# quantumjot/sequitr

Hardware: AMD Instinct MI355X
Metric: segmented Mpixels/sec on 512x512 tiles; IoU vs reference (higher is better)
Workload: dtype f32; 1 GPU; U-Net 2-class inference, launches of 32 512x512x1 tiles, fp32 (BASELINE.json configs[1]: filters 16-32-64-128-256, eltwise_mul bridge); logits + uint8 argmax mask; one 32-tile batch per GPU per step; tiles_this_rank=32

## Files before the change

include/sequitr_hip.h:

```cpp
#ifndef SEQUITR_HIP_H
#define SEQUITR_HIP_H

#include <stdint.h>

#ifdef __cplusplus
extern "C" {
#endif

#define SQ_OK 0
#define SQ_EINVAL (-1)
#define SQ_ELAUNCH (-2)
#define SQ_EALIGN (-3)

#define SQ_ACT_NONE 0
#define SQ_ACT_RELU 1
#define SQ_ACT_LEAKY 2

#define SQ_BRIDGE_NONE 0
#define SQ_BRIDGE_ADD 1
#define SQ_BRIDGE_MUL 2
#define SQ_BRIDGE_SUB 3

int sq_version(void);
const char *sq_last_error(void);
// ... 276 lines not shown

int64_t sq_weightmap_workspace(int N, int H, int W);
int sq_edt_sq_f32(const float *img, int32_t *d2, void *workspace, int N, int H, int W, void *stream);
int sq_weightmap_edt_f32(const float *img, double *out64, float *out32, void *workspace, int N, int H, int W,
                         double w0, double sigma, void *stream);

int64_t sq_weightmap2_workspace(int N, int H, int W);
int sq_wm2_boundary_points_u8(const float *img, uint8_t *points, int N, int H, int W, void *stream);
int64_t sq_delaunay2d_batch_i32(const int32_t *xy, const int64_t *offsets, int nsets, int32_t *simplices, double *longest,
                                int64_t cap);
int sq_weightmap2_delaunay_f32(const float *img, const int32_t *simplices, const double *longest, int nsimp, double *out64,
                               float *out32, void *workspace, int N, int H, int W, double w0, double sigma, void *stream);

int sq_pixelnorm_fwd_bf16(const void *x, void *y, int64_t npix, int C, float eps, void *stream);
int sq_pixelnorm_bwd_bf16(const void *x, const void *dy, void *dx, int64_t npix, int C, float eps, int act, void *stream);
int sq_pixelnorm_bwd2_bf16(const void *x, const void *g, const void *v, void *dg, void *dx2, int64_t npix, int C, float eps,
                           void *stream);
int sq_sumpool2x2_bf16(const void *x, void *y, int N, int H, int W, int C, float scale, void *stream);
int sq_broadcast2x2_bf16(const void *src, void *dst, int N, int H, int W, int C, float scale, void *stream);
int sq_broadcast2x2_act_bwd_bf16(const void *src, const void *gate, void *dst, int N, int H, int W, int C, float scale,
                                 int act, void *stream);
int sq_act_fwd_bf16(const void *x, void *y, int64_t n, int act, void *stream);
int sq_conv1x1_smallin_fwd_bf16(const float *x, const float *w, const float *bias, void *y, int64_t npix, int Ca, int C,
                                float wscale, int act, void *stream);
int sq_conv1x1_smallout_fwd_bf16(const void *x, const float *w, const float *bias, float *y, int64_t npix, int C, int Co,
                                 float wscale, int act, void *stream);
int64_t sq_wgrad1x1_small_workspace_bf16(int64_t npix, int Ca, int C);
int sq_wgrad1x1_small_bf16(const float *a, const void *b, float *m, float *asum, float *workspace, int64_t npix, int Ca,
                           int C, float scale, void *stream);
int sq_conv2d_nhwc_fwd_avgpool_bf16(const void *x, const void *wp, const float *bias, void *y, void *ypool, int N, int H, int W,
                                    int Cin, int Cout, int act, void *stream);
int sq_conv2d_nhwc_fwd_pixelnorm_bf16(const void *x, const void *wp, const float *bias, void *y, void *ynorm, int N, int H, int W,
                                      int Cin, int Cout, int act, float eps, void *stream);
int sq_conv2d_nhwc_dgrad_actgate_bf16(const void *dy, const void *wp_t, const void *gate, int act, void *dx, int N, int H,
                                      int W, int Cin, int Cout, int K, void *stream);
int sq_conv2d_nhwc_mosaic_bf16(const void *x, const void *wp, const float *bias, const void *gate, void *y, int Nimg, int h,
                               int w, int Cin, int Cout, int act, int R, int Cc, float *workspace, int64_t workspace_bytes,
                               void *stream);
#define SQ_PLAN_BF16 0
#define SQ_PLAN_MIXED 1
#define SQ_PLAN_F32 2
#define SQ_PLAN_PLAIN 0
#define SQ_PLAN_JUNCTION 1
#define SQ_PLAN_POOL 2
#define SQ_PLAN_MASK 3
#define SQ_PLAN_MASKGATE 4
#define SQ_PLAN_ACTGATE 5
#define SQ_PLAN_FIRSTBLOCK 8
#define SQ_PLAN_PIXELNORM 9
#define SQ_PLAN_CONCAT 10
#define SQ_PLAN_WSCALE 1
int sq_conv_plan(int family, int form, int N, int H, int W, int Cin, int Cout, int K, int act, int flags, const int *mosaic,
                 int64_t workspace_bytes, int *out);
int sq_conv2d_nhwc_wgrad_scaled_bf16(const void *x, const void *dy, float *dw, float *db, float *workspace, int N, int H,
                                     int W, int Cin, int Cout, int K, float dw_scale, void *stream);
int sq_conv2d_nhwc_wgrad_mosaic_bf16(const void *x, const void *dy, float *dw, float *db, float *workspace, int Nimg, int h,
                                     int w, int Cin, int Cout, int R, int Cc, float dw_scale, void *stream);

typedef struct sq_wgrad_item {
    const void *x, *dy;
    float *dw, *db;
    int32_t N, H, W, Cin, Cout, K;
    int32_t convT_cout;
    float dw_scale;
    int32_t accumulate;
    int32_t mosaic_R, mosaic_Cc;
    int32_t reserved;
} sq_wgrad_item;
int64_t sq_conv2d_nhwc_wgrad_group_workspace_bf16(const sq_wgrad_item *items, int n);
int sq_conv2d_nhwc_wgrad_group_bf16(const sq_wgrad_item *items, int n, float *workspace, void *stream);

#define SQ_WGP_KS 0
#define SQ_WGP_NI 1
#define SQ_WGP_NO 2
#define SQ_WGP_KIND 3
#define SQ_WGP_PF 4
#define SQ_WGP_NPAIRS 5
#define SQ_WGP_GX 6
#define SQ_WGP_TPB 7
#define SQ_WGP_G 8
#define SQ_WGP_WS 9
#define SQ_WGP_N 10
#define SQ_WGP_GROUP_N (SQ_WGP_N + 3)
#define SQ_WGP_PLAIN 0
#define SQ_WGP_MOSAIC 1
#define SQ_WGP_RAGGED 2
#define SQ_WGP_CONVT 3
#define SQ_WGP_F32 4
#define SQ_WGP_F32_SMALL 5
int sq_wgrad_plan(int family, int N, int H, int W, int Cin, int Cout, int K, const int *mosaic, int convT_cout, int64_t *out);
int sq_wgrad_group_plan(const sq_wgrad_item *items, int n, int64_t *out);

#define SQ_C3P_KIND 0
#define SQ_C3P_BN 1
#define SQ_C3P_KC 2
#define SQ_C3P_GX 3
#define SQ_C3P_GY 4
#define SQ_C3P_ADDR 5
#define SQ_C3P_N 6
#define SQ_C3_MFMA 0
#define SQ_C3_DIRECT 1
#define SQ_C3_FLAT 0
#define SQ_C3_WINDOW 1
int sq_conv3d_plan(int N, int D, int H, int W, int Cin, int Cout, int *out);
int sq_conv3d_ndhwc_fwd_f32(const float *x, const float *w, const float *bias, float *y, int N, int D, int H, int W,
                            int Cin, int Cout, int act, void *stream);
// ... 20 lines not shown
```

sequitr_amd/_lib.py:

```python
import ctypes
import os

_HERE = os.path.dirname(os.path.abspath(__file__))
LIB_PATH = os.path.join(_HERE, "_build", "libsequitr_hip.so")

c_void_p, c_int, c_float, c_int64 = ctypes.c_void_p, ctypes.c_int, ctypes.c_float, ctypes.c_int64


class WgradItem(ctypes.Structure):
    _fields_ = [("x", c_void_p), ("dy", c_void_p), ("dw", c_void_p), ("db", c_void_p),
                ("N", ctypes.c_int32), ("H", ctypes.c_int32), ("W", ctypes.c_int32), ("Cin", ctypes.c_int32),
                ("Cout", ctypes.c_int32), ("K", ctypes.c_int32), ("convT_cout", ctypes.c_int32), ("dw_scale", c_float),
                ("accumulate", ctypes.c_int32), ("mosaic_R", ctypes.c_int32), ("mosaic_Cc", ctypes.c_int32),
                ("reserved", ctypes.c_int32)]

SIGNATURES = {
    "sq_version": (c_int, []),
    "sq_last_error": (ctypes.c_char_p, []),
    "sq_conv2d_nhwc_fwd_f32": (c_int, [c_void_p] * 4 + [c_int] * 6 + [c_float, c_int, c_void_p]),
    "sq_maxpool2x2_fwd_f32": (c_int, [c_void_p] * 2 + [c_int] * 4 + [c_void_p]),
    "sq_avgpool2x2_fwd_f32": (c_int, [c_void_p] * 2 + [c_int] * 4 + [c_void_p]),
    "sq_convT2x2s2_nhwc_fwd_f32": (c_int, [c_void_p] * 5 + [c_int] * 6 + [c_void_p]),
    "sq_bridge_fwd_f32": (c_int, [c_void_p] * 3 + [c_int64, c_int, c_void_p]),
    "sq_conv1x1_argmax_fwd_f32": (c_int, [c_void_p] * 5 + [c_int] * 5 + [c_void_p]),
# ... 93 lines not shown
    "sq_conv2d_nhwc_wgrad_workspace_mixed_f32": (c_int64, [c_int] * 6),
    "sq_conv2d_nhwc_wgrad_mixed_f32": (c_int, [c_void_p] * 5 + [c_int] * 6 + [c_void_p]),
    "sq_conv2d_nhwc_wgrad_scaled_mixed_f32": (c_int, [c_void_p] * 5 + [c_int] * 6 + [c_float, c_void_p]),
    "sq_conv2d_nhwc_wgrad_scaled_f32": (c_int, [c_void_p] * 5 + [c_int] * 6 + [c_float, c_void_p]),
    "sq_conv3x3_first_fwd_bf16": (c_int, [c_void_p] * 4 + [c_int] * 6 + [c_void_p]),
    "sq_conv2d_nhwc_wgrad_workspace_bf16": (c_int64, [c_int] * 6),
    "sq_conv2d_nhwc_wgrad_bf16": (c_int, [c_void_p] * 5 + [c_int] * 6 + [c_void_p]),
    "sq_convT2x2s2_wgrad_bf16": (c_int, [c_void_p] * 5 + [c_int] * 5 + [c_void_p]),
    "sq_cast_f32_to_bf16": (c_int, [c_void_p] * 2 + [c_int64, c_void_p]),
    "sq_cast_bf16_to_f32": (c_int, [c_void_p] * 2 + [c_int64, c_void_p]),
    "sq_head_concat_fwd_bf16": (c_int, [c_void_p] * 3 + [c_int64, c_int, c_void_p]),
    "sq_head_concat_bwd_bf16": (c_int, [c_void_p] * 3 + [c_int64, c_int, c_void_p]),
    "sq_maxpool2x2_fwd_bf16": (c_int, [c_void_p] * 2 + [c_int] * 4 + [c_void_p]),
    "sq_maxpool2x2_bwd_bf16": (c_int, [c_void_p] * 3 + [c_int] * 4 + [c_void_p]),
    "sq_conv_pack_weights_multi_bf16": (c_int, [c_void_p, c_void_p, c_void_p, c_int, c_int, c_void_p]),
    "sq_conv_pack_weights_multi_scaled_bf16": (c_int, [c_void_p] * 4 + [c_int, c_int, c_void_p]),
    "sq_conv2d_nhwc_fwd_dropout_bf16": (c_int, [c_void_p] * 4 + [c_int] * 7 + [c_float, ctypes.c_uint32, c_void_p, c_void_p]),
    "sq_conv3x3_first_fwd_mask_bf16": (c_int, [c_void_p] * 5 + [c_int] * 6 + [c_void_p]),
    "sq_conv2d_nhwc_fwd_mask_bf16": (c_int, [c_void_p] * 5 + [c_int] * 7 + [c_void_p]),
    "sq_conv2d_nhwc_dgrad_maskgate_bf16": (c_int, [c_void_p] * 3 + [c_float, c_void_p] + [c_int] * 6 + [c_void_p]),
    "sq_conv2d_nhwc_wgrad_mixed_mosaic_f32": (c_int, [c_void_p] * 5 + [c_int] * 7 + [c_float, c_void_p]),
    "sq_conv2d_nhwc_mixed_mosaic_f32": (c_int, [c_void_p] * 5 + [c_int] * 8 + [c_void_p]),
    "sq_conv2d_nhwc_dgrad_actgate_mixed_f32": (c_int, [c_void_p] * 3 + [c_int, c_void_p] + [c_int] * 6 + [c_void_p]),
    "sq_conv2d_nhwc_fwd_dropout_pool_bf16": (c_int, [c_void_p] * 5 + [c_int] * 7 + [c_float, ctypes.c_uint32, c_void_p, c_void_p]),
    "sq_conv3x3_first_block_dropout_pool_bf16": (c_int, [c_void_p] * 9 + [c_int] * 3 + [c_float, ctypes.c_uint32, c_void_p, c_void_p]),
    "sq_relu_scale_bwd_bf16": (c_int, [c_void_p] * 3 + [c_int64, c_float, c_void_p]),
    "sq_bridge_bwd_s2d_bf16": (c_int, [c_void_p] * 5 + [c_int] * 5 + [c_void_p]),
    "sq_maxpool2x2_bwd_add_bf16": (c_int, [c_void_p] * 4 + [c_int] * 4 + [c_void_p]),
    "sq_maxpool2x2_bwd_add_gate_bf16": (c_int, [c_void_p] * 4 + [c_int] * 4 + [c_float, c_void_p]),
    "sq_conv2d_nhwc_dgrad_gate_bf16": (c_int, [c_void_p] * 3 + [c_float, c_void_p] + [c_int] * 6 + [c_void_p]),
    "sq_conv2d_nhwc_dgrad_junction_bf16": (c_int, [c_void_p] * 6 + [c_int] * 7 + [c_void_p]),
    "sq_conv1x1_head_bwd_gate_bf16": (c_int, [c_void_p] * 7 + [c_int64, c_int, c_int, c_float, c_void_p]),
    "sq_conv1x1_head_wce_fwd_bf16": (c_int, [c_void_p] * 7 + [c_int64, c_int, c_int, c_void_p]),
    "sq_conv1x1_head_wce_bwd_bf16": (c_int, [c_void_p] * 10 + [c_int64, c_int, c_int, c_float, c_void_p]),
    "sq_conv1x1_head_wce_bwd_loss_bf16": (c_int, [c_void_p] * 12 + [c_int64, c_int, c_int, c_float, c_void_p]),
    "sq_act_dropout_bwd_bf16": (c_int, [c_void_p] * 4 + [c_int64, c_float, c_int, c_void_p]),
    "sq_conv2d_nhwc_dgrad_relu_bf16": (c_int, [c_void_p] * 4 + [c_int] * 6 + [c_void_p]),
    "sq_pixelnorm_fwd_bf16": (c_int, [c_void_p] * 2 + [c_int64, c_int, c_float, c_void_p]),
    "sq_pixelnorm_bwd_bf16": (c_int, [c_void_p] * 3 + [c_int64, c_int, c_float, c_int, c_void_p]),
    "sq_pixelnorm_bwd2_bf16": (c_int, [c_void_p] * 5 + [c_int64, c_int, c_float, c_void_p]),
    "sq_sumpool2x2_bf16": (c_int, [c_void_p] * 2 + [c_int] * 4 + [c_float, c_void_p]),
    "sq_broadcast2x2_bf16": (c_int, [c_void_p] * 2 + [c_int] * 4 + [c_float, c_void_p]),
    "sq_broadcast2x2_act_bwd_bf16": (c_int, [c_void_p] * 3 + [c_int] * 4 + [c_float, c_int, c_void_p]),
    "sq_act_fwd_bf16": (c_int, [c_void_p] * 2 + [c_int64, c_int, c_void_p]),
    "sq_conv1x1_smallin_fwd_bf16": (c_int, [c_void_p] * 4 + [c_int64, c_int, c_int, c_float, c_int, c_void_p]),
    "sq_conv1x1_smallout_fwd_bf16": (c_int, [c_void_p] * 4 + [c_int64, c_int, c_int, c_float, c_int, c_void_p]),
    "sq_wgrad1x1_small_workspace_bf16": (c_int64, [c_int64, c_int, c_int]),
    "sq_wgrad1x1_small_bf16": (c_int, [c_void_p] * 5 + [c_int64, c_int, c_int, c_float, c_void_p]),
    "sq_conv2d_nhwc_fwd_avgpool_bf16": (c_int, [c_void_p] * 5 + [c_int] * 6 + [c_void_p]),
    "sq_conv2d_nhwc_fwd_pixelnorm_bf16": (c_int, [c_void_p] * 5 + [c_int] * 6 + [c_float, c_void_p]),
    "sq_conv2d_nhwc_dgrad_actgate_bf16": (c_int, [c_void_p] * 3 + [c_int, c_void_p] + [c_int] * 6 + [c_void_p]),
    "sq_conv2d_nhwc_mosaic_bf16": (c_int, [c_void_p] * 5 + [c_int] * 8 + [c_void_p, c_int64, c_void_p]),
    "sq_conv_plan": (c_int, [c_int] * 10 + [c_void_p, c_int64, c_void_p]),
    "sq_conv2d_nhwc_wgrad_scaled_bf16": (c_int, [c_void_p] * 5 + [c_int] * 6 + [c_float, c_void_p]),
    "sq_conv2d_nhwc_wgrad_mosaic_bf16": (c_int, [c_void_p] * 5 + [c_int] * 7 + [c_float, c_void_p]),
    "sq_conv2d_nhwc_wgrad_group_workspace_bf16": (c_int64, [c_void_p, c_int]),
    "sq_conv2d_nhwc_wgrad_group_bf16": (c_int, [c_void_p, c_int, c_void_p, c_void_p]),
    "sq_wgrad_plan": (c_int, [c_int] * 7 + [c_void_p, c_int, c_void_p]),
    "sq_wgrad_group_plan": (c_int, [c_void_p, c_int, c_void_p]),
    "sq_conv3d_plan": (c_int, [c_int] * 6 + [c_void_p]),
    "sq_conv3d_ndhwc_fwd_f32": (c_int, [c_void_p] * 4 + [c_int] * 7 + [c_void_p]),
    "sq_maxpool2x2x2_fwd_f32": (c_int, [c_void_p] * 2 + [c_int] * 5 + [c_void_p]),
    "sq_convT2x2x2s2_ndhwc_fwd_f32": (c_int, [c_void_p] * 5 + [c_int] * 7 + [c_void_p]),
    "sq_act_bwd_bf16": (c_int, [c_void_p] * 3 + [c_int64, c_int, c_void_p]),
    "sq_bridge_fwd_bf16": (c_int, [c_void_p] * 3 + [c_int64, c_int, c_void_p]),
    "sq_bridge_bwd_bf16": (c_int, [c_void_p] * 5 + [c_int64, c_int, c_void_p]),
    "sq_dropout_fwd_bf16": (c_int, [c_void_p] * 3 + [c_int64, c_float, ctypes.c_uint32, c_int, c_void_p, c_void_p]),
    "sq_dropout_bwd_bf16": (c_int, [c_void_p] * 3 + [c_int64, c_float, c_void_p]),
    "sq_convT2x2s2_nhwc_fwd_bf16": (c_int, [c_void_p] * 5 + [c_int] * 6 + [c_void_p]),
    "sq_convT2x2s2_bridge_both_fwd_bf16": (c_int, [c_void_p] * 6 + [c_int] * 6 + [c_void_p]),
    "sq_conv1x1_head_fwd_bf16": (c_int, [c_void_p] * 5 + [c_int64, c_int, c_int, c_void_p]),
    "sq_conv1x1_head_bwd_workspace_bf16": (c_int64, [c_int64, c_int, c_int]),
    "sq_conv1x1_head_bwd_bf16": (c_int, [c_void_p] * 7 + [c_int64, c_int, c_int, c_void_p]),
    "sq_conv3x3_first_wgrad_workspace_bf16": (c_int64, [c_int] * 5),
    "sq_conv3x3_first_wgrad_bf16": (c_int, [c_void_p] * 5 + [c_int] * 5 + [c_void_p]),
}

_lib = None


class SequitrHipError(RuntimeError):
    pass


def load():
    global _lib
    if _lib is not None:
        return _lib
    if not os.path.exists(LIB_PATH):
        raise SequitrHipError(
            "libsequitr_hip.so not found at %s -- the HIP back end is mandatory "
            "(no CPU fallback); build it with `make -C sequitr_amd/csrc`" % LIB_PATH)
    import torch
    lib = ctypes.CDLL(LIB_PATH)
    for name, (res, args) in SIGNATURES.items():
        try:
            fn = getattr(lib, name)
        except AttributeError:
            raise SequitrHipError("libsequitr_hip.so does not export %s" % name)
        fn.restype = res
        fn.argtypes = args
    _lib = lib
    return lib


def check(rc, name):
# ... 4 lines not shown
```

sequitr_amd/csrc/sq_common.h:

```cpp
#pragma once
#include <hip/hip_runtime.h>
#include <stdint.h>
#include <stdio.h>
#include "../../include/sequitr_hip.h"

typedef float f32x4 __attribute__((ext_vector_type(4)));

#define SQ_NOT_MINE 1

void sq_set_error(const char *fmt, ...);

#define SQ_REQUIRE(cond, ...)            \
    do {                                 \
        if (!(cond)) {                   \
            sq_set_error(__VA_ARGS__);   \
            return SQ_EINVAL;            \
        }                                \
    } while (0)

int sq_plan_bf16_kc(int Cin);
int sq_plan_bf16_bn(int64_t ntiles, int Cout, bool pn, bool mos);
int sq_plan_mosaic_splitk(int Nimg, int h, int w, int Cin, int Cout, int R, int Cc, bool have_ws, int64_t workspace_bytes);
int sq_plan_f32_bn(int64_t ntiles, int Cout);
bool sq_plan_f32_stage32(int bn, int KS, int KC, int Cin, bool concat);
bool sq_plan_l0_takes(int mode, int cout, int act, int H, int W, bool concat, int head_c, bool pooled);
int sq_wgrad_f32_plan(int N, int H, int W, int Cin, int Cout, int K, int64_t *out);

#define SQ_ALIGNED16(p) ((((uintptr_t)(p)) & 15u) == 0)

#define SQ_REQUIRE_ALIGNED(p)                                     \
    do {                                                          \
        if (!SQ_ALIGNED16(p)) {                                   \
            sq_set_error("%s: pointer %s not 16-byte aligned", __func__, #p); \
            return SQ_EALIGN;                                     \
        }                                                         \
    } while (0)

static inline int sq_check_launch(const char *what) {
    hipError_t e = hipGetLastError();
    if (e != hipSuccess) {
        sq_set_error("%s: launch failed: %s", what, hipGetErrorString(e));
        return SQ_ELAUNCH;
    }
    return SQ_OK;
}

__device__ __forceinline__ float sq_act(float v, int act) {
    if (act == SQ_ACT_RELU) return v > 0.0f ? v : 0.0f;
    if (act == SQ_ACT_LEAKY) return v > 0.0f ? v : 0.2f * v;
    return v;
}

__device__ __forceinline__ unsigned sq_xcd_remap(unsigned bid, unsigned nblk) {
    const unsigned q = nblk >> 3, r = nblk & 7u, xcd = bid & 7u, k = bid >> 3;
    const unsigned base = xcd < r ? xcd * (q + 1) : r * (q + 1) + (xcd - r) * q;
    return base + k;
}

struct SqDropKey { unsigned s1, s2; };
__device__ __forceinline__ SqDropKey sq_dropout_key(unsigned seed, const int *__restrict__ step) {
    if (step) seed += (unsigned)step[0] * 0x9E3779B9u;
    SqDropKey k;
    k.s1 = seed * 0x9E3779B1u + 0x7F4A7C15u;
    k.s2 = (seed ^ 0x68E31DA4u) * 0x85EBCA6Bu;
    k.s2 ^= k.s2 >> 13;
    return k;
}
__device__ __forceinline__ unsigned sq_dropout_thr16(float rate) { return (unsigned)(rate * 65536.0f); }
__device__ __forceinline__ unsigned sq_dropout_keep4(SqDropKey k, unsigned q, unsigned thr16) {
    unsigned h = q + k.s1;
    h ^= h >> 16; h *= 0x7FEB352Du; h = h ^ (h >> 15) ^ k.s2; h *= 0x846CA68Bu; h ^= h >> 16;
    unsigned g = (h ^ 0x5BD1E995u) * 0x2C1B3C6Du;
    g ^= g >> 15;
    return (unsigned)((h & 0xFFFFu) >= thr16) | ((unsigned)((h >> 16) >= thr16) << 1) |
           ((unsigned)((g & 0xFFFFu) >= thr16) << 2) | ((unsigned)((g >> 16) >= thr16) << 3);
}

template <int MAXC>
// ... 44 lines not shown
```

sequitr_amd/csrc/sq_conv_epi.h:

```cpp
#pragma once
#include "sq_common.h"

struct SqConvEpi {
    float *pooled;
    const float *head_w;
    const float *head_b;
    float *logits;
    uint8_t *mask;
    int head_c;
    int store_y;
    const float *first_w;
    const float *first_b;
    const float *up_x;
    const float *up_w;
    const float *up_b;
    int up_bridge;
    const float *x2;
};

#define SQ_L0_NOT_MINE 1
int sq_conv_l0_launch(int mode, const float *x, const float *w, const float *bias, float *y, int N, int H, int W,
                      int cout, int act, const SqConvEpi &epi, hipStream_t st);
```

sequitr_amd/csrc/sq_conv_f32_v2.hip:

```cpp
#include <stdlib.h>
#include <type_traits>
#include "sq_common.h"
#include "sq_conv_epi.h"

#ifndef SQ_V2_FAST32
#define SQ_V2_FAST32 1
#endif
#ifndef SQ_V2_INNER
#define SQ_V2_INNER 1
#endif
#ifndef SQ_TILE_INTERLEAVE
#define SQ_TILE_INTERLEAVE 1
#endif
#ifndef SQ_STORE_PERMUTE
#define SQ_STORE_PERMUTE 0
#endif


namespace {

constexpr int TH = 16, TW = 16;

template <int BN, int KS, int KC>
struct Cfg2 {
// ... 541 lines not shown
                epilogue(ctx, cty, cn, std::integral_constant<bool, false>{});
            }
        }
        if (has_next) __syncthreads();
        if (ntile != tile) {
            ctx = ntx; cty = nty; cn = nn;
            ntx += s_x;
            if (ntx >= tiles_x) { ntx -= tiles_x; nty += 1; }
            nty += s_y;
            if (nty >= tiles_y) { nty -= tiles_y; nn += 1; }
            nn += s_n;
        }
        tile = ntile;
        chunk = nchk;
    }
}

template <int BN, int KS, int KC, int MODE>
int launch_v2(const float *x, const float *w, const float *bias, float *y, int N, int H, int W, int Cin,
              int Cout, float wscale, int act, const SqConvEpi &epi, hipStream_t st) {
    using C = Cfg2<BN, KS, KC>;
    static bool attr_set = false;
    auto kern = conv_mfma_f32_v2_kernel<BN, KS, KC, MODE>;
    constexpr int lds_base = MODE == 1 ? C::LDS_BYTES_FIRST : (MODE == 2 ? C::LDS_BYTES_UP : C::LDS_BYTES);
    constexpr int lds_max = lds_base + C::HEAD_FLOATS * 4;
    const int lds = lds_base + (epi.head_w ? C::HEAD_FLOATS * 4 : 0);
    if (!attr_set) {
        if (hipFuncSetAttribute(reinterpret_cast<const void *>(kern),
                                hipFuncAttributeMaxDynamicSharedMemorySize, lds_max) != hipSuccess) {
            sq_set_error("conv_mfma_f32_v2: cannot reserve %d bytes of LDS", lds_max);
            return SQ_ELAUNCH;
        }
        attr_set = true;
    }
    const int tiles_x = (W + TW - 1) / TW, tiles_y = (H + TH - 1) / TH;
    const int ntiles = tiles_x * tiles_y * N;
    const int gy = (Cout + BN - 1) / BN;
    int want = (256 * (MODE == 2 ? 3 : C::OCC) + gy - 1) / gy;
    if (want < 1) want = 1;
    int tpb = (ntiles + want - 1) / want;
    if (tpb < 1) tpb = 1;
    const int gx = (ntiles + tpb - 1) / tpb;
    hipLaunchKernelGGL(kern, dim3(gx, gy), dim3(256), lds, st, x, w, bias, y, N, H, W, Cin, Cout,
                       wscale, act, tiles_x, tiles_y, ntiles, tpb, epi);
    return sq_check_launch("sq_conv2d_nhwc_fwd_f32(v2)");
}

template <int KS, int KC>
int dispatch_bn(const float *x, const float *w, const float *bias, float *y, int N, int H, int W, int Cin,
                int Cout, float wscale, int act, const SqConvEpi &epi, hipStream_t st) {
    const int ntiles = ((W + TW - 1) / TW) * ((H + TH - 1) / TH) * N;
    const int bn = sq_plan_f32_bn(ntiles, Cout);
    if constexpr (KS == 3 && KC == 16) {
        if (sq_plan_f32_stage32(bn, KS, KC, Cin, epi.x2 != nullptr))
            return launch_v2<32, 3, 32, false>(x, w, bias, y, N, H, W, Cin, Cout, wscale, act, epi, st);
    }
    if (bn == 64) return launch_v2<64, KS, KC, false>(x, w, bias, y, N, H, W, Cin, Cout, wscale, act, epi, st);
    if (bn == 32) return launch_v2<32, KS, KC, false>(x, w, bias, y, N, H, W, Cin, Cout, wscale, act, epi, st);
    return launch_v2<16, KS, KC, false>(x, w, bias, y, N, H, W, Cin, Cout, wscale, act, epi, st);
}

bool fits32(int N, int H, int W, int C) { return (size_t)N * H * W * (size_t)C * 4 < ((size_t)1 << 31); }

}

int sq_conv_mfma_v2(const float *x, const float *w, const float *bias, float *y, int N, int H, int W,
                    int Cin, int Cout, int K, float wscale, int act, hipStream_t st) {
    SqConvEpi epi = {};
    epi.store_y = 1;
    if (Cin == 16 && (Cout == 16 || Cout == 32) && K == 3 && wscale == 1.0f) {
        const int r = sq_conv_l0_launch(0, x, w, bias, y, N, H, W, Cout, act, epi, st);
        if (r != SQ_L0_NOT_MINE) return r;
    }
    if (Cin % 16 == 0)
        return K == 3 ? dispatch_bn<3, 16>(x, w, bias, y, N, H, W, Cin, Cout, wscale, act, epi, st)
                      : dispatch_bn<1, 16>(x, w, bias, y, N, H, W, Cin, Cout, wscale, act, epi, st);
    return K == 3 ? dispatch_bn<3, 8>(x, w, bias, y, N, H, W, Cin, Cout, wscale, act, epi, st)
                  : dispatch_bn<1, 8>(x, w, bias, y, N, H, W, Cin, Cout, wscale, act, epi, st);
}

extern "C" int sq_conv2d_concat_nhwc_fwd_f32(const float *xa, const float *xb, const float *w, const float *bias, float *y,
                                             int N, int H, int W, int Ca, int Cout, int K, int act, void *stream) {
    SQ_REQUIRE(xa && xb && w && y, "sq_conv2d_concat_nhwc_fwd_f32: null tensor pointer");
    SQ_REQUIRE(N > 0 && H > 0 && W > 0 && (K == 1 || K == 3), "sq_conv2d_concat_nhwc_fwd_f32: bad shape / K");
    SQ_REQUIRE(Ca % 16 == 0 && Ca > 0 && Cout % 4 == 0 && Cout > 0,
               "sq_conv2d_concat_nhwc_fwd_f32: channels per source %d (multiple of 16), Cout=%d (multiple of 4)", Ca, Cout);
    SQ_REQUIRE(fits32(N, H, W, 2 * Ca > Cout ? 2 * Ca : Cout), "sq_conv2d_concat_nhwc_fwd_f32: tensors must be < 2 GiB");
    SQ_REQUIRE(act >= SQ_ACT_NONE && act <= SQ_ACT_LEAKY, "sq_conv2d_concat_nhwc_fwd_f32: bad activation %d", act);
    SQ_REQUIRE_ALIGNED(xa); SQ_REQUIRE_ALIGNED(xb); SQ_REQUIRE_ALIGNED(w); SQ_REQUIRE_ALIGNED(y);
    if (bias) SQ_REQUIRE_ALIGNED(bias);
    SqConvEpi epi = {};
    epi.store_y = 1;
    epi.x2 = xb;
    hipStream_t st = reinterpret_cast<hipStream_t>(stream);
    return K == 3 ? dispatch_bn<3, 16>(xa, w, bias, y, N, H, W, 2 * Ca, Cout, 1.0f, act, epi, st)
                  : dispatch_bn<1, 16>(xa, w, bias, y, N, H, W, 2 * Ca, Cout, 1.0f, act, epi, st);
}

extern "C" int sq_conv3x3_pool_fwd_f32(const float *x, const float *w, const float *bias, float *y, float *pooled,
                                       int N, int H, int W, int Cin, int Cout, int act, void *stream) {
    SQ_REQUIRE(x && w && y && pooled, "sq_conv3x3_pool_fwd_f32: null tensor pointer");
    SQ_REQUIRE(N > 0 && H > 0 && W > 0 && H % 2 == 0 && W % 2 == 0, "sq_conv3x3_pool_fwd_f32: H, W must be even");
    SQ_REQUIRE(Cin % 16 == 0 && Cin > 0 && Cout % 4 == 0 && Cout > 0,
               "sq_conv3x3_pool_fwd_f32: Cin=%d (multiple of 16), Cout=%d (multiple of 4)", Cin, Cout);
    SQ_REQUIRE(fits32(N, H, W, Cin > Cout ? Cin : Cout), "sq_conv3x3_pool_fwd_f32: tensors must be < 2 GiB");
    SQ_REQUIRE(act >= SQ_ACT_NONE && act <= SQ_ACT_LEAKY, "sq_conv3x3_pool_fwd_f32: bad activation %d", act);
// ... 77 lines not shown
```

sequitr_amd/csrc/sq_conv_plan.hip:

```cpp
#include "sq_conv_epi.h"
#include <stdlib.h>

namespace {
constexpr int TILE = 16;
int64_t ntiles_of(int N, int H, int W) { return (int64_t)((W + TILE - 1) / TILE) * ((H + TILE - 1) / TILE) * N; }
}

int sq_plan_bf16_kc(int Cin) { return Cin % 32 == 0 ? 32 : (Cin % 16 == 0 ? 16 : 8); }

int sq_plan_bf16_bn(int64_t ntiles, int Cout, bool pn, bool mos) {
    if (pn) return Cout <= 16 ? 16 : (Cout <= 32 ? 32 : 64);
    int bn = Cout >= 64 ? 64 : (Cout > 16 ? 32 : 16);
    static const int narrow = [] { const char *e = getenv("SQ_CONV_BF16_NARROW"); return e ? atoi(e) : 1; }();
    while (narrow && bn > 16 && ntiles * ((Cout + bn - 1) / bn) < 2 * 256) bn >>= 1;
    static const int force_bn = [] { const char *e = getenv("SQ_MOS_BN"); return e ? atoi(e) : 0; }();
    if (mos && (force_bn == 16 || force_bn == 32 || force_bn == 64) && force_bn <= ((Cout + 15) / 16) * 16) bn = force_bn;
    return bn;
}

int sq_plan_mosaic_splitk(int Nimg, int h, int w, int Cin, int Cout, int R, int Cc, bool have_ws, int64_t workspace_bytes) {
    const int H = R * (h + 1), W = Cc * (w + 1);
    const int nchunk = Cin / sq_plan_bf16_kc(Cin);
    const int64_t blocks = ntiles_of(1, H, W) * ((Cout + 15) / 16);
    const int64_t slice = (int64_t)Nimg * h * w * Cout * 4;
    int S = 1;
    static const int sk_on = [] { const char *e = getenv("SQ_CONV_SPLITK"); return e ? atoi(e) : 1; }();
    if (sk_on && have_ws && Cout % 4 == 0 && blocks < 256 && nchunk >= 4)
        while (S < 8 && nchunk % (2 * S) == 0 && nchunk / (2 * S) >= 2 && blocks * S < 512 && slice * 2 * S <= workspace_bytes) S *= 2;
    static const int force_s = [] { const char *e = getenv("SQ_MOS_S"); return e ? atoi(e) : 0; }();
    if (force_s >= 1 && have_ws && nchunk % force_s == 0 && slice * force_s <= workspace_bytes) S = force_s;
    return S;
}

int sq_plan_f32_bn(int64_t ntiles, int Cout) {
    int bn = Cout >= 64 ? 64 : (Cout > 16 ? 32 : 16);
    while (bn > 16 && ntiles * ((Cout + bn - 1) / bn) < 2 * 256) bn >>= 1;
    return bn;
}

bool sq_plan_f32_stage32(int bn, int KS, int KC, int Cin, bool concat) {
    static const bool on = [] { const char *e = getenv("SQ_CONV_STAGE32"); return !(e && e[0] == '0'); }();
    return KS == 3 && KC == 16 && bn == 32 && Cin % 32 == 0 && !concat && on;
}

bool sq_plan_l0_takes(int mode, int cout, int act, int H, int W, bool concat, int head_c, bool pooled) {
    if (cout != 16 && !(cout == 32 && mode == 0 && !head_c && !pooled)) return false;
    const char *e = getenv("SQ_CONV_L0");
    if (e && e[0] == '0') return false;
    if (act != SQ_ACT_RELU || H % 16 != 0 || W % 16 != 0 || concat) return false;
    if (head_c && head_c != 2) return false;
    if (head_c && pooled) return false;
    return true;
}

extern "C" int sq_conv_plan(int family, int form, int N, int H, int W, int Cin, int Cout, int K, int act, int flags,
                            const int *mosaic, int64_t workspace_bytes, int *out) {
    SQ_REQUIRE(out, "sq_conv_plan: null out");
    SQ_REQUIRE(N > 0 && H > 0 && W > 0 && Cin > 0 && Cout > 0 && (K == 1 || K == 3), "sq_conv_plan: bad shape / K");
    SQ_REQUIRE(act >= SQ_ACT_NONE && act <= SQ_ACT_LEAKY, "sq_conv_plan: bad activation %d", act);
    out[0] = out[1] = out[2] = 0;
    out[3] = 1;
    out[4] = 0;
    if (family == SQ_PLAN_F32) {
        SQ_REQUIRE(!mosaic, "sq_conv_plan: the f32 family has no mosaic form");
        SQ_REQUIRE(Cout % 4 == 0 && (Cin % 16 == 0 || (Cin == 8 && form == SQ_PLAN_PLAIN)),
                   "sq_conv_plan: the f32 v2 kernels take Cin %% 16 == 0 (or 8, plain), Cout %% 4 == 0");
        SQ_REQUIRE(form == SQ_PLAN_PLAIN || form == SQ_PLAN_CONCAT || (form == SQ_PLAN_POOL && K == 3),
                   "sq_conv_plan: f32 form %d at K=%d does not exist", form, K);
        const bool wscale1 = !(flags & SQ_PLAN_WSCALE);
        const bool offer = form == SQ_PLAN_PLAIN ? (Cin == 16 && (Cout == 16 || Cout == 32) && K == 3 && wscale1)
                                                 : (form == SQ_PLAN_POOL && Cin == 16 && Cout == 16);
        if (offer && sq_plan_l0_takes(0, Cout, act, H, W, false, 0, form == SQ_PLAN_POOL)) {
            out[0] = Cout;
            out[1] = 16;
            out[2] = 1;
            out[4] = 1;
            return SQ_OK;
        }
        const int KC = Cin % 16 == 0 ? 16 : 8;
        const int bn = sq_plan_f32_bn(ntiles_of(N, H, W), Cout);
        const bool s32 = sq_plan_f32_stage32(bn, K, KC, Cin, form == SQ_PLAN_CONCAT);
        out[0] = bn;
        out[1] = s32 ? 32 : KC;
        out[2] = (Cout + bn - 1) / bn;
        return SQ_OK;
    }
    SQ_REQUIRE(family == SQ_PLAN_BF16 || family == SQ_PLAN_MIXED, "sq_conv_plan: bad family %d", family);
    SQ_REQUIRE(Cin % 8 == 0 && Cout % 4 == 0, "sq_conv_plan: Cin=%d (multiple of 8), Cout=%d (multiple of 4)", Cin, Cout);
    const bool bf = family == SQ_PLAN_BF16;
    int NN = N, HH = H, WW = W;
    if (mosaic) {
        SQ_REQUIRE(K == 3 && (form == SQ_PLAN_PLAIN || form == SQ_PLAN_ACTGATE), "sq_conv_plan: the mosaic forms are 3x3 plain / act-gated");
        SQ_REQUIRE(mosaic[0] > 0 && mosaic[1] > 0 && (int64_t)mosaic[0] * mosaic[1] >= N && H <= 8 && W <= 8,
                   "sq_conv_plan: mosaic of R x Cc >= Nimg cells of images up to 8 x 8");
        NN = 1;
        HH = mosaic[0] * (H + 1);
        WW = mosaic[1] * (W + 1);
        if (bf) out[3] = sq_plan_mosaic_splitk(N, H, W, Cin, Cout, mosaic[0], mosaic[1], workspace_bytes > 0, workspace_bytes);
    } else {
        switch (form) {
        case SQ_PLAN_PLAIN: case SQ_PLAN_ACTGATE: break;
        case SQ_PLAN_POOL: case SQ_PLAN_JUNCTION:
            SQ_REQUIRE(bf && K == 3, "sq_conv_plan: form %d is a 3x3 form on bf16 tensors", form); break;
        case SQ_PLAN_MASK: case SQ_PLAN_MASKGATE:
            SQ_REQUIRE(bf && K == 3 && Cout % 16 == 0, "sq_conv_plan: the mask forms are 3x3, Cout %% 16 == 0, bf16 tensors"); break;
// ... 15 lines not shown
```

Before: 1650 Mpixels/s.

## Add persistent wide-tile f32 MFMA conv kernel for 3x3 Cin=32 layers

Adds a new persistent f32 3x3 convolution kernel using 16x16 spatial tiles with an 18x18 halo in LDS. It double-buffers the next tile's halo and weight chunk in registers while the current tile runs MFMA, and can fuse a 2x2 max-pool into the epilogue. By default it only handles layers where the planner picks BN=32 and Cin=32; other shapes fall back to the existing v2 kernels. The goal is better input reuse and less launch and prologue overhead per tile. The cost is high register pressure from holding the full 3x3 filter slice per lane, plus a new planner path gated by an environment variable.

```diff
diff --git a/include/sequitr_hip.h b/include/sequitr_hip.h
--- a/include/sequitr_hip.h
+++ b/include/sequitr_hip.h
@@ -352,6 +352,7 @@
 #define SQ_PLAN_WSCALE 1
 int sq_conv_plan(int family, int form, int N, int H, int W, int Cin, int Cout, int K, int act, int flags, const int *mosaic,
                  int64_t workspace_bytes, int *out);
+int sq_conv_wide_plan(int N, int H, int W, int Cin, int Cout, int K, int act, int form, int *out);
 int sq_conv2d_nhwc_wgrad_scaled_bf16(const void *x, const void *dy, float *dw, float *db, float *workspace, int N, int H,
                                      int W, int Cin, int Cout, int K, float dw_scale, void *stream);
 int sq_conv2d_nhwc_wgrad_mosaic_bf16(const void *x, const void *dy, float *dw, float *db, float *workspace, int Nimg, int h,
diff --git a/sequitr_amd/_lib.py b/sequitr_amd/_lib.py
--- a/sequitr_amd/_lib.py
+++ b/sequitr_amd/_lib.py
@@ -169,6 +169,7 @@
     "sq_conv2d_nhwc_dgrad_actgate_bf16": (c_int, [c_void_p] * 3 + [c_int, c_void_p] + [c_int] * 6 + [c_void_p]),
     "sq_conv2d_nhwc_mosaic_bf16": (c_int, [c_void_p] * 5 + [c_int] * 8 + [c_void_p, c_int64, c_void_p]),
     "sq_conv_plan": (c_int, [c_int] * 10 + [c_void_p, c_int64, c_void_p]),
+    "sq_conv_wide_plan": (c_int, [c_int] * 8 + [c_void_p]),
     "sq_conv2d_nhwc_wgrad_scaled_bf16": (c_int, [c_void_p] * 5 + [c_int] * 6 + [c_float, c_void_p]),
     "sq_conv2d_nhwc_wgrad_mosaic_bf16": (c_int, [c_void_p] * 5 + [c_int] * 7 + [c_float, c_void_p]),
     "sq_conv2d_nhwc_wgrad_group_workspace_bf16": (c_int64, [c_void_p, c_int]),
diff --git a/sequitr_amd/csrc/sq_common.h b/sequitr_amd/csrc/sq_common.h
--- a/sequitr_amd/csrc/sq_common.h
+++ b/sequitr_amd/csrc/sq_common.h
@@ -24,6 +24,8 @@
 int sq_plan_f32_bn(int64_t ntiles, int Cout);
 bool sq_plan_f32_stage32(int bn, int KS, int KC, int Cin, bool concat);
 bool sq_plan_l0_takes(int mode, int cout, int act, int H, int W, bool concat, int head_c, bool pooled);
+int sq_plan_wide_bn(int N, int H, int W, int Cin, int Cout, int K, int act, bool concat, bool wscale1, bool pooled);
+void sq_plan_wide_grid(int64_t ntiles, int bn, int Cout, int *gx, int *gy);
 int sq_wgrad_f32_plan(int N, int H, int W, int Cin, int Cout, int K, int64_t *out);
 
 #define SQ_ALIGNED16(p) ((((uintptr_t)(p)) & 15u) == 0)
diff --git a/sequitr_amd/csrc/sq_conv_epi.h b/sequitr_amd/csrc/sq_conv_epi.h
--- a/sequitr_amd/csrc/sq_conv_epi.h
+++ b/sequitr_amd/csrc/sq_conv_epi.h
@@ -21,3 +21,8 @@
 #define SQ_L0_NOT_MINE 1
 int sq_conv_l0_launch(int mode, const float *x, const float *w, const float *bias, float *y, int N, int H, int W,
                       int cout, int act, const SqConvEpi &epi, hipStream_t st);
+
+#define SQ_WIDE_OCC64 2
+#define SQ_WIDE_OCC32 2
+int sq_conv_wide_launch(const float *x, const float *w, const float *bias, float *y, float *pooled, int N, int H, int W,
+                        int Cin, int Cout, int K, int act, bool concat, bool wscale1, hipStream_t st);
diff --git a/sequitr_amd/csrc/sq_conv_f32_v2.hip b/sequitr_amd/csrc/sq_conv_f32_v2.hip
--- a/sequitr_amd/csrc/sq_conv_f32_v2.hip
+++ b/sequitr_amd/csrc/sq_conv_f32_v2.hip
@@ -617,6 +617,11 @@
     const int ntiles = ((W + TW - 1) / TW) * ((H + TH - 1) / TH) * N;
     const int bn = sq_plan_f32_bn(ntiles, Cout);
     if constexpr (KS == 3 && KC == 16) {
+        const int r = sq_conv_wide_launch(x, w, bias, y, epi.pooled, N, H, W, Cin, Cout, KS, act, epi.x2 != nullptr,
+                                          wscale == 1.0f, st);
+        if (r != SQ_NOT_MINE) return r;
+    }
+    if constexpr (KS == 3 && KC == 16) {
         if (sq_plan_f32_stage32(bn, KS, KC, Cin, epi.x2 != nullptr))
             return launch_v2<32, 3, 32, false>(x, w, bias, y, N, H, W, Cin, Cout, wscale, act, epi, st);
     }
diff --git a/sequitr_amd/csrc/sq_conv_f32_wide.hip b/sequitr_amd/csrc/sq_conv_f32_wide.hip
--- /dev/null
+++ b/sequitr_amd/csrc/sq_conv_f32_wide.hip
@@ -0,0 +1,292 @@
+#include <stdlib.h>
+#include "sq_common.h"
+#include "sq_conv_epi.h"
+
+namespace {
+
+constexpr int TH = 16, TW = 16, HWD = 18, HP = HWD * HWD;
+constexpr int PS = 24;
+constexpr int XS_FLOATS = HP * PS;
+constexpr unsigned OOB = 0x80000000u;
+
+enum { EPI_STORE = 0, EPI_POOL = 1 };
+
+struct WArgs {
+    const float *x, *w, *bias;
+    float *y, *pooled;
+    int N, H, W, Cin, Cout, nchunk;
+    int tiles_x, tiles_y, ntiles;
+    int gx, gy, gn;
+};
+
+typedef unsigned u32x4 __attribute__((__vector_size__(4 * sizeof(unsigned))));
+
+template <int ACT>
+__device__ __forceinline__ float act_of(float v) {
+    if constexpr (ACT == SQ_ACT_RELU) return __builtin_fmaxf(v, 0.0f);
+    else if constexpr (ACT == SQ_ACT_LEAKY) return v > 0.0f ? v : v * 0.2f;
+    else return v;
+}
+
+template <int BN>
+constexpr int wide_occ() { return BN == 64 ? SQ_WIDE_OCC64 : SQ_WIDE_OCC32; }
+
+template <int BN, int EPI, int ACT, int NCI>
+__global__ __launch_bounds__(256, wide_occ<BN>()) void conv_wide_kernel(const WArgs a) {
+    constexpr int QPP = 4 * NCI;
+    constexpr int XITEMS = HP * QPP, XSLOTS = (XITEMS + 255) / 256;
+    constexpr int NG = BN / 16;
+    constexpr int RW = 16 * NG / 4;
+    constexpr int HR = RW + 2;
+    extern __shared__ __attribute__((aligned(16))) float xs[];
+
+    const int tid = threadIdx.x, lane = tid & 63, wv = tid >> 6;
+    const int li = lane & 15, kk = lane >> 4;
+    const int grp = wv % NG, band = wv / NG;
+    const int co0 = blockIdx.y * BN + 16 * grp;
+    const int H = a.H, W = a.W, Cin = a.Cin, Cout = a.Cout;
+    const int G = (int)gridDim.x;
+    const int vb = (int)sq_xcd_remap(blockIdx.x, gridDim.x);
+    if (vb >= a.ntiles) return;
+    const int t_count = (a.ntiles - vb + G - 1) / G;
+    const int nchunk = a.nchunk / NCI, nitems = t_count * nchunk;
+
+    const __amdgpu_buffer_rsrc_t xrsrc = __builtin_amdgcn_make_buffer_rsrc(
+        const_cast<float *>(a.x), 0, (int)((size_t)a.N * H * W * Cin * 4), 0x00020000);
+    const __amdgpu_buffer_rsrc_t wrsrc = __builtin_amdgcn_make_buffer_rsrc(
+        const_cast<float *>(a.w), 0, 9 * Cin * Cout * 4, 0x00020000);
+    const __amdgpu_buffer_rsrc_t yrsrc = __builtin_amdgcn_make_buffer_rsrc(
+        a.y, 0, (int)((size_t)a.N * H * W * Cout * 4), 0x00020000);
+    const int Hl = H >> 1, Wl = W >> 1;
+    const __amdgpu_buffer_rsrc_t prsrc = __builtin_amdgcn_make_buffer_rsrc(
+        a.pooled, 0, EPI == EPI_POOL ? (int)((size_t)a.N * Hl * Wl * Cout * 4) : 0, 0x00020000);
+
+    const float4 bv = a.bias ? *reinterpret_cast<const float4 *>(a.bias + co0 + 4 * kk) : make_float4(-0.f, -0.f, -0.f, -0.f);
+
+    float af[NCI][9][4], an[9][4];
+    const int wlane = (kk * Cout + co0 + li) * 4;
+    const int wstep_s = 16 * Cout, wstep_t = (Cin - 12) * Cout * 4;
+    auto issue_w = [&](int cc) {
+        int off = 16 * cc * Cout * 4;
+#pragma unroll
+        for (int t = 0; t < 9; ++t)
+#pragma unroll
+            for (int s = 0; s < 4; ++s) {
+                an[t][s] = __builtin_bit_cast(float, __builtin_amdgcn_raw_buffer_load_b32(wrsrc, wlane, off, 0));
+                off += s < 3 ? wstep_s : wstep_t;
+            }
+    };
+
+    float4 xr[XSLOTS];
+    int xrel[XSLOTS], xpp[XSLOTS];
+#pragma unroll
+    for (int sl = 0; sl < XSLOTS; ++sl) {
+        const int idx = tid + sl * 256, pix = idx / QPP, q = idx % QPP;
+        const int py = pix / HWD, px = pix % HWD;
+        xrel[sl] = idx < XITEMS ? ((py * W + px) * Cin + q * 4) * 4 : (int)OOB;
+        xpp[sl] = (py << 8) | px;
+    }
+    auto issue_halo = [&](int tx, int ty, int n, int cc) {
+        const int x0 = tx * TW - 1, y0 = ty * TH - 1;
+        const int base = (((n * H + y0) * W + x0) * Cin + 16 * cc) * 4;
+        if (tx > 0 && tx < a.tiles_x - 1 && ty > 0 && ty < a.tiles_y - 1) {
+#pragma unroll
+            for (int sl = 0; sl < XSLOTS; ++sl) {
+                const auto v = __builtin_amdgcn_raw_buffer_load_b128(xrsrc, xrel[sl], base, 0);
+                xr[sl] = *reinterpret_cast<const float4 *>(&v);
+            }
+        } else {
+#pragma unroll
+            for (int sl = 0; sl < XSLOTS; ++sl) {
+                const int py = xpp[sl] >> 8, px = xpp[sl] & 255;
+                const bool inb = (unsigned)(y0 + py) < (unsigned)H && (unsigned)(x0 + px) < (unsigned)W && xrel[sl] != (int)OOB;
+                const unsigned off = inb ? (unsigned)(base + xrel[sl]) : OOB;
+                const auto v = __builtin_amdgcn_raw_buffer_load_b128(xrsrc, off, 0, 0);
+                xr[sl] = *reinterpret_cast<const float4 *>(&v);
+            }
+        }
+    };
+    float *cw = xs + (tid % QPP / 4) * XS_FLOATS + (tid / QPP) * PS + (tid & 3);
+    auto commit = [&]() {
+#pragma unroll
+        for (int sl = 0; sl < XSLOTS; ++sl) {
+            if (sl < XSLOTS - 1 || tid < XITEMS - (XSLOTS - 1) * 256) {
+                float *d = cw + sl * (256 / QPP) * PS;
+                d[0] = xr[sl].x; d[4] = xr[sl].y; d[8] = xr[sl].z; d[12] = xr[sl].w;
+            }
+        }
+        if constexpr (NCI == 1) {
+#pragma unroll
+            for (int t = 0; t < 9; ++t)
+#pragma unroll
+                for (int s = 0; s < 4; ++s) af[0][t][s] = an[t][s];
+        }
+    };
+
+    f32x4 acc[RW];
+#pragma unroll
+    for (int r = 0; r < RW; ++r) acc[r] = (f32x4){0.f, 0.f, 0.f, 0.f};
+    const float *xb0 = xs + ((RW * band) * HWD + li) * PS + 4 * kk;
+    auto mfma_phase = [&](const float *xb, const float (&fa)[9][4]) {
+        float4 bq[2][3];
+#pragma unroll
+        for (int kx = 0; kx < 3; ++kx) bq[0][kx] = *reinterpret_cast<const float4 *>(xb + kx * PS);
+        __builtin_amdgcn_s_setprio(0);
+#pragma unroll
+        for (int h = 0; h < HR; ++h) {
+            if (h + 1 < HR) {
+#pragma unroll
+                for (int kx = 0; kx < 3; ++kx)
+                    bq[(h + 1) & 1][kx] = *reinterpret_cast<const float4 *>(xb + ((h + 1) * HWD + kx) * PS);
+            }
+            __builtin_amdgcn_sched_barrier(0);
+#pragma unroll
+            for (int kx = 0; kx < 3; ++kx) {
+                const float4 q = bq[h & 1][kx];
+                const float b[4] = {q.x, q.y, q.z, q.w};
+#pragma unroll
+                for (int s = 0; s < 4; ++s) {
+#pragma unroll
+                    for (int ky = 2; ky >= 0; --ky) {
+                        const int r = h - ky;
+                        if (r < 0 || r >= RW) continue;
+                        acc[r] = __builtin_amdgcn_mfma_f32_16x16x4f32(fa[ky * 3 + kx][s], b[s], acc[r], 0, 0, 0);
+                    }
+                }
+            }
+            __builtin_amdgcn_sched_barrier(0);
+        }
+        __builtin_amdgcn_s_setprio(3);
+    };
+
+    const int yvoff = (((RW * band) * W + li) * Cout + co0 + 4 * kk) * 4;
+    const int pvoff = (((RW / 2 * band) * Wl + (li >> 1)) * Cout + co0 + 4 * kk) * 4;
+    auto epilogue = [&](int tx, int ty, int n) {
+        const int tbase = (((n * H + ty * TH) * W + tx * TW) * Cout) * 4;
+        const int pbase = (((n * Hl + ty * (TH / 2)) * Wl + tx * (TW / 2)) * Cout) * 4;
+#pragma unroll
+        for (int r = 0; r < RW; r += 2) {
+            f32x4 o[2];
+#pragma unroll
+            for (int u = 0; u < 2; ++u) {
+                o[u] = (f32x4){act_of<ACT>(acc[r + u][0] + bv.x), act_of<ACT>(acc[r + u][1] + bv.y),
+                               act_of<ACT>(acc[r + u][2] + bv.z), act_of<ACT>(acc[r + u][3] + bv.w)};
+                __builtin_amdgcn_raw_buffer_store_b128(*reinterpret_cast<const u32x4 *>(&o[u]), yrsrc,
+                                                       yvoff + tbase + (r + u) * W * Cout * 4, 0, 0);
+                acc[r + u] = (f32x4){0.f, 0.f, 0.f, 0.f};
+            }
+            if constexpr (EPI == EPI_POOL) {
+                f32x4 mp;
+#pragma unroll
+                for (int j = 0; j < 4; ++j) {
+                    const float t0 = o[0][j], t1 = o[1][j];
+                    const float v = ACT == SQ_ACT_RELU ? __builtin_fmaxf(t0, t1) : (t1 > t0 ? t1 : t0);
+                    const float u = __builtin_bit_cast(float, __builtin_amdgcn_mov_dpp(__builtin_bit_cast(int, v), 0xB1, 0xF, 0xF, true));
+                    mp[j] = ACT == SQ_ACT_RELU ? __builtin_fmaxf(u, v) : (u > v ? u : v);
+                }
+                __builtin_amdgcn_raw_buffer_store_b128(*reinterpret_cast<const u32x4 *>(&mp), prsrc,
+                                                       (li & 1) ? (int)OOB : pvoff + pbase + (r / 2) * Wl * Cout * 4, 0, 0);
+            }
+        }
+    };
+
+    int ctx = vb % a.tiles_x, cty = (vb / a.tiles_x) % a.tiles_y, cn = vb / (a.tiles_x * a.tiles_y);
+    int ntx = ctx + a.gx, nty = cty, nn = cn;
+    if (ntx >= a.tiles_x) { ntx -= a.tiles_x; nty += 1; }
+    nty += a.gy;
+    if (nty >= a.tiles_y) { nty -= a.tiles_y; nn += 1; }
+    nn += a.gn;
+    issue_halo(ctx, cty, cn, 0);
+    if constexpr (NCI == 1) issue_w(0);
+    else {
+#pragma unroll
+        for (int c = 0; c < NCI; ++c) {
+            issue_w(c);
+            __builtin_amdgcn_s_waitcnt(0x0F70);
+#pragma unroll
+            for (int t = 0; t < 9; ++t)
+#pragma unroll
+                for (int s = 0; s < 4; ++s) af[c][t][s] = an[t][s];
+        }
+    }
+    __builtin_amdgcn_s_waitcnt(0x0F70);
+    commit();
+    __syncthreads();
+    int chunk = 0;
+    for (int it = 0; it < nitems; ++it) {
+        const bool has_next = it + 1 < nitems;
+        const bool last = chunk == nchunk - 1;
+        const int nchk = last ? 0 : chunk + 1;
+        if (has_next) {
+            if (last) issue_halo(ntx, nty, nn, 0);
+            else issue_halo(ctx, cty, cn, nchk);
+            if (NCI == 1 && nchunk > 1) issue_w(nchk);
+        }
+#pragma unroll
+        for (int c = 0; c < NCI; ++c) mfma_phase(xb0 + c * XS_FLOATS, af[c]);
+        __builtin_amdgcn_s_waitcnt(0x0F70);
+        if (has_next) {
+            __syncthreads();
+            commit();
+        }
+        if (last) {
+            epilogue(ctx, cty, cn);
+            ctx = ntx; cty = nty; cn = nn;
+            ntx += a.gx;
+            if (ntx >= a.tiles_x) { ntx -= a.tiles_x; nty += 1; }
+            nty += a.gy;
+            if (nty >= a.tiles_y) { nty -= a.tiles_y; nn += 1; }
+            nn += a.gn;
+        }
+        if (has_next) __syncthreads();
+        chunk = nchk;
+    }
+}
+
+template <int BN, int EPI, int ACT, int NCI>
+int launch_wide(const WArgs &a0, int gx, int gy, hipStream_t st) {
+    static bool attr_set = false;
+    auto kern = conv_wide_kernel<BN, EPI, ACT, NCI>;
+    constexpr int lds = NCI * XS_FLOATS * 4;
+    if (!attr_set) {
+        if (hipFuncSetAttribute(reinterpret_cast<const void *>(kern), hipFuncAttributeMaxDynamicSharedMemorySize, lds) != hipSuccess) {
+            sq_set_error("conv_wide: cannot reserve %d bytes of LDS", lds);
+            return SQ_ELAUNCH;
+        }
+        attr_set = true;
+    }
+    WArgs a = a0;
+    const int per_image = a.tiles_x * a.tiles_y;
+    a.gn = gx / per_image;
+    a.gy = (gx % per_image) / a.tiles_x;
+    a.gx = (gx % per_image) % a.tiles_x;
+    hipLaunchKernelGGL(kern, dim3(gx, gy), dim3(256), lds, st, a);
+    return sq_check_launch("conv_wide");
+}
+
+template <int BN, int EPI, int NCI = 1>
+int launch_act(const WArgs &a, int act, int gx, int gy, hipStream_t st) {
+    if (act == SQ_ACT_RELU) return launch_wide<BN, EPI, SQ_ACT_RELU, NCI>(a, gx, gy, st);
+    if (act == SQ_ACT_LEAKY) return launch_wide<BN, EPI, SQ_ACT_LEAKY, NCI>(a, gx, gy, st);
+    return launch_wide<BN, EPI, SQ_ACT_NONE, NCI>(a, gx, gy, st);
+}
+
+}
+
+int sq_conv_wide_launch(const float *x, const float *w, const float *bias, float *y, float *pooled, int N, int H, int W,
+                        int Cin, int Cout, int K, int act, bool concat, bool wscale1, hipStream_t st) {
+    const int bn = sq_plan_wide_bn(N, H, W, Cin, Cout, K, act, concat, wscale1, pooled != nullptr);
+    if (!bn) return SQ_NOT_MINE;
+    WArgs a = {};
+    a.x = x; a.w = w; a.bias = bias; a.y = y; a.pooled = pooled;
+    a.N = N; a.H = H; a.W = W; a.Cin = Cin; a.Cout = Cout; a.nchunk = Cin / 16;
+    a.tiles_x = W / TW;
+    a.tiles_y = H / TH;
+    a.ntiles = a.tiles_x * a.tiles_y * N;
+    int gx = 0, gy = 0;
+    sq_plan_wide_grid(a.ntiles, bn, Cout, &gx, &gy);
+    if (bn == 64) return pooled ? launch_act<64, EPI_POOL>(a, act, gx, gy, st) : launch_act<64, EPI_STORE>(a, act, gx, gy, st);
+    if (Cin == 32)
+        return pooled ? launch_act<32, EPI_POOL, 2>(a, act, gx, gy, st) : launch_act<32, EPI_STORE, 2>(a, act, gx, gy, st);
+    return pooled ? launch_act<32, EPI_POOL>(a, act, gx, gy, st) : launch_act<32, EPI_STORE>(a, act, gx, gy, st);
+}
diff --git a/sequitr_amd/csrc/sq_conv_plan.hip b/sequitr_amd/csrc/sq_conv_plan.hip
--- a/sequitr_amd/csrc/sq_conv_plan.hip
+++ b/sequitr_amd/csrc/sq_conv_plan.hip
@@ -51,6 +51,41 @@
     if (head_c && head_c != 2) return false;
     if (head_c && pooled) return false;
     return true;
+}
+
+int sq_plan_wide_bn(int N, int H, int W, int Cin, int Cout, int K, int act, bool concat, bool wscale1, bool pooled) {
+    const char *e = getenv("SQ_CONV_WIDE");
+    const int mode = e ? atoi(e) : 1;
+    if (mode == 0) return 0;
+    if (K != 3 || concat || !wscale1 || act < SQ_ACT_NONE || act > SQ_ACT_LEAKY) return 0;
+    if (Cin < 32 || Cin % 16 != 0 || H % 16 != 0 || W % 16 != 0) return 0;
+    (void)pooled;
+    const int bn = sq_plan_f32_bn(ntiles_of(N, H, W), Cout);
+    if (bn < 32 || Cout % bn != 0) return 0;
+    if (mode == 1 && !(bn == 32 && Cin == 32)) return 0;
+    return bn;
+}
+
+void sq_plan_wide_grid(int64_t ntiles, int bn, int Cout, int *gx, int *gy) {
+    *gy = Cout / bn;
+    const int64_t want = (256 * (bn == 64 ? SQ_WIDE_OCC64 : SQ_WIDE_OCC32) + *gy - 1) / *gy;
+    *gx = (int)(ntiles < want ? ntiles : want);
+}
+
+extern "C" int sq_conv_wide_plan(int N, int H, int W, int Cin, int Cout, int K, int act, int form, int *out) {
+    SQ_REQUIRE(out, "sq_conv_wide_plan: null out");
+    SQ_REQUIRE(N > 0 && H > 0 && W > 0 && Cin > 0 && Cout > 0 && (K == 1 || K == 3), "sq_conv_wide_plan: bad shape / K");
+    SQ_REQUIRE(act >= SQ_ACT_NONE && act <= SQ_ACT_LEAKY, "sq_conv_wide_plan: bad activation %d", act);
+    SQ_REQUIRE(form == SQ_PLAN_PLAIN || form == SQ_PLAN_CONCAT || (form == SQ_PLAN_POOL && K == 3),
+               "sq_conv_wide_plan: f32 form %d at K=%d does not exist", form, K);
+    out[0] = out[1] = out[2] = out[3] = out[4] = 0;
+    const int bn = sq_plan_wide_bn(N, H, W, Cin, Cout, K, act, form == SQ_PLAN_CONCAT, true, form == SQ_PLAN_POOL);
+    if (!bn) return SQ_OK;
+    out[0] = 1;
+    out[1] = bn;
+    out[2] = 16;
+    sq_plan_wide_grid(ntiles_of(N, H, W), bn, Cout, &out[3], &out[4]);
+    return SQ_OK;
 }
 
 extern "C" int sq_conv_plan(int family, int form, int N, int H, int W, int Cin, int Cout, int K, int act, int flags,
```

Result: no change. 1664 Mpixels/s, median of 6 (+0.9%).
